# YJxyzxyz/road-vision-system

Measured on AMD Instinct MI355X. Metric: end-to-end frames/sec @1080p (preproc+YOLOv8n+SORT), 1/2/4/8 MI355X, higher is better.
Workload: dtype bf16

## Files before the change

### include/rvhip.h

```cpp
#ifndef RVHIP_H
#define RVHIP_H

#include <stddef.h>
#include <stdint.h>

#ifdef __cplusplus
extern "C" {
#endif

#define RV_OK 0
#define RV_EINVAL (-1000)
#define RV_ECAP (-1001)
#define RV_EOF 1

int rv_abi_version(void);
const char* rv_last_error(void);
int rv_trace_marker(int tag, void* stream);
int rv_install_crash_handler(void);


size_t rv_clahe_ws_bytes(int B, int tiles);

int rv_clahe_ycrcb_u8(const uint8_t* in, uint8_t* out, int B, int H, int W,
                      int pitch, int tiles, double clip, void* ws,
// ... 99 lines not shown
int rv_yolo_pack2(int variant, int dtype, const float* flat, size_t n, void* host_out,
                  size_t out_bytes);
int rv_yolo_create2(int variant, int dtype, const void* dev_packed, int max_B, int in_h, int in_w,
                    void** handle);

int rv_yolo_num_convs_nc(int variant, int nc);
int rv_yolo_conv_info_nc(int variant, int nc, int idx, int* info, char* name, int name_cap);
size_t rv_yolo_flat_floats_nc(int variant, int nc);
size_t rv_yolo_packed_bytes3(int variant, int dtype, int nc);
int rv_yolo_pack3(int variant, int dtype, int nc, const float* flat, size_t n, void* host_out,
                  size_t out_bytes);
int rv_yolo_create3(int variant, int dtype, int nc, const void* dev_packed, int max_B, int in_h,
                    int in_w, void** handle);
int rv_yolo_num_classes(void* handle);
int rv_yolo_head_form(void* handle);
int rv_yolo_set_act_scales(void* handle, const float* scales, int n);
int rv_yolo_buffer_esize(void* handle, int buf);
int rv_yolo_buffer_name(void* handle, int buf, char* name, int cap);
float rv_fp8_scale(double amax);
size_t rv_yolo_ws_bytes(void* handle, int B);
int rv_yolo_num_anchors(void* handle);
int rv_yolo_cand_segments(void* handle);
int rv_yolo_forward(void* handle, const uint8_t* lb, int B, void* ws, size_t ws_bytes,
                    float* raw_out, float conf, void* cand, int cand_cap, int* cand_n,
                    void* stream);
int rv_yolo_forward_part(void* handle, const uint8_t* lb, int B, void* ws, size_t ws_bytes,
                         float* raw_out, float conf, void* cand, int cand_cap, int* cand_n,
                         void* stream, int part);

int rv_yolo_num_buffers(void* handle);
int rv_yolo_buffer_info(void* handle, int B, int buf, int* info, size_t* off_bytes);
int rv_yolo_trace(void* handle, int* recs, int max_recs);
int rv_yolo_attn_trace(void* handle, int* recs, int max_recs);

int rv_yolo_profile(void* handle, int max_forwards);
int rv_yolo_profile_reps(void* handle, int max_forwards, int reps);
int rv_yolo_profile_read(void* handle, double* ms, double* flops, int* conv, int n);
int rv_yolo_profile_bytes(void* handle, double* bytes, int n);
int rv_yolo_profile_times(void* handle, void* ref, double* t0, double* t1, int n);

int rv_yolo_autotune(void* handle, const uint8_t* lb, int B, void* ws, size_t ws_bytes,
                     int reps, int verify, int* n_bad, void* stream);
int rv_yolo_tuned_config(void* handle, int idx, int* cfg6);
int rv_yolo_set_tuned(void* handle, int n, int idx, const int* cfg6);
int rv_yolo_conv_candidates(void* handle, int idx, int* cfg6, int cap);

size_t rv_nms_smem_bytes(void);
int rv_nms_postprocess(const void* cand, const int* seg_n, int B, int cap, int nseg,
                       float iou, int max_det, int max_nms, float max_wh, const float* scale5,
                       const uint32_t* keep_mask4, float* out, int* out_n, int* cand_total,
                       void* ws, size_t ws_bytes, void* stream);
size_t rv_nms_ws_bytes(int B);
int rv_cand_segments(int A);
int rv_candidates_from_raw(const float* raw, int B, int nc, int A, float conf, void* cand,
                           int cap, int* seg_n, void* stream);

size_t rv_sort_state_bytes(int S, int tmax);
size_t rv_sort_ws_bytes(int S, int tmax, int dmax);
int rv_sort_init(void* state, int S, int tmax, void* stream);
int rv_sort_update(void* state_in, void* state_out, int S, int tmax, const float* dets,
                   const int* dcount, int dmax, const double* ts, const double* params6,
                   const double* H9, const float* origin2, void* ws, size_t ws_bytes,
                   int* out_id, double* out_dist, double* out_speed, void* stream);
int rv_sort_stats(const void* state, int S, int* T_out, int* next_id_out, int* overflow_out,
                  void* stream);
int rv_sort_export(const void* state, int S, int tmax, double* x_out, int* meta, int* T_out,
// ... 177 lines not shown
```

### road-vision-system_amd/csrc/c2f.hip

```cpp
#include "conv.h"
#include "conv_common.h"

namespace rv {

typedef __attribute__((ext_vector_type(8))) __bf16 bf16x8c;
typedef __attribute__((ext_vector_type(4))) float f32x4c;
typedef __attribute__((ext_vector_type(2))) float f32x2c;
typedef __attribute__((ext_vector_type(2))) __bf16 bf16x2c;

__device__ __forceinline__ uint32_t c2f_pack(float lo, float hi) {
  return __builtin_bit_cast(uint32_t, __builtin_convertvector(f32x2c{lo, hi}, bf16x2c));
}
__device__ __forceinline__ float c2f_bf2f(uint32_t h) { return __uint_as_float(h << 16); }

template <int C>
struct C2fGeo {
  static constexpr int PB = 2 * C;
  static constexpr int NQ = PB / 16;
  static constexpr int MR = C / 16;
  __device__ static __forceinline__ int addr(int p, int q) { return p * PB + (q << 4); }
};

template <int TR, int TC>
struct C2fTile {
  __host__ __device__ static constexpr int rh(int e) { return TR + 2 * e; }
  __host__ __device__ static constexpr int rw(int e) { return TC + 2 * e; }
  __host__ __device__ static constexpr int rp(int e) { return rh(e) * rw(e); }
};

template <int C, int N, int TR, int TC>
struct C2fLds {
  using G = C2fGeo<C>;
  using T = C2fTile<TR, TC>;
  static constexpr int h = 2 * N;
  static constexpr int Y = 0;
  static constexpr int Tb = Y + T::rp(h) * G::PB;
  static constexpr int Z0 = Tb + T::rp(h - 1) * G::PB;
  static constexpr int Z1 = Z0 + T::rp(h - 2) * G::PB;
  static constexpr int Y0 = Z1 + (N == 2 ? T::rp(0) * G::PB : 0);
  static constexpr int ZR = Y0 + T::rp(0) * G::PB;
  static constexpr int ZBYTES = G::NQ < 4 ? (2 * T::rw(h) + 3) * G::PB : 0;
  static constexpr int BYTES = ZR + ZBYTES;
};

template <int C, int TR, int TC, bool RES, int EO, int ER>
__device__ __forceinline__ void c2f_conv3(const uint8_t* __restrict__ in, uint8_t* __restrict__ outb,
                                          const bf16_t* __restrict__ w,
                                          const float* __restrict__ bias,
                                          const uint8_t* __restrict__ res, int oy0, int ox0, int H,
                                          int W, const uint8_t* __restrict__ zeros, bool pairs) {
  using G = C2fGeo<C>;
  using T = C2fTile<TR, TC>;
  constexpr int MR = G::MR;
  const int tid = threadIdx.x, wave = tid >> 6, lane = tid & 63;
  const int col = lane & 15, quad = lane >> 4;
  constexpr int e_out = EO, e_res = ER;
  constexpr int rwo = T::rw(e_out), rpo = T::rp(e_out), rwi = rwo + 2, rwr = T::rw(e_res);
  bf16x8c A[9][MR];
#pragma unroll
  for (int t = 0; t < 9; ++t)
#pragma unroll
    for (int m = 0; m < MR; ++m)
      A[t][m] = __builtin_bit_cast(bf16x8c,
                                   *(const uint4*)(w + ((size_t)(m * 16 + col) * 9 + t) * 32 + quad * 8));
  f32x4c bv[MR];
#pragma unroll
  for (int m = 0; m < MR; ++m) bv[m] = *(const f32x4c*)(bias + m * 16 + quad * 4);
  const int nfrag = (rpo + 15) / 16;
  if (C == 16 && pairs) {
    bf16x8c Ap[5];
#pragma unroll
    for (int p = 0; p < 5; ++p) {
      const int t = 2 * p + (quad >> 1);
      uint4 v = make_uint4(0, 0, 0, 0);
      if (t < 9) v = *(const uint4*)(w + ((size_t)col * 9 + t) * 32 + (quad & 1) * 8);
      Ap[p] = __builtin_bit_cast(bf16x8c, v);
    }
    const bool hiq = quad >= 2;
    for (int f0 = wave * 2; f0 < nfrag; f0 += 16) {
      f32x4c acc[2];
      int o[2];
      const uint8_t* b1[2];
      const uint8_t* b2[2];
      const uint8_t* b4[2];
#pragma unroll
      for (int n = 0; n < 2; ++n) {
        o[n] = (f0 + n) * 16 + col;
        const int oo = o[n] < rpo ? o[n] : 0;
        const int r = oo / rwo, c = oo - r * rwo;
        const uint8_t* bp = in + G::addr(r * rwi + c, quad & 1);
        b1[n] = bp + (hiq ? G::PB : 0);
        b2[n] = bp + (hiq ? (rwi - 2) * G::PB : 0) + (2 * G::PB);
        b4[n] = hiq ? zeros : bp + (2 * rwi + 2) * G::PB;
        acc[n] = f32x4c{0.f, 0.f, 0.f, 0.f};
      }
      bf16x8c Bp[5][2];
#pragma unroll
      for (int n = 0; n < 2; ++n) {
        Bp[0][n] = __builtin_bit_cast(bf16x8c, *(const uint4*)(b1[n]));
        Bp[1][n] = __builtin_bit_cast(bf16x8c, *(const uint4*)(b2[n]));
        Bp[2][n] = __builtin_bit_cast(bf16x8c, *(const uint4*)(b1[n] + (rwi + 1) * G::PB));
        Bp[3][n] = __builtin_bit_cast(bf16x8c, *(const uint4*)(b1[n] + (2 * rwi) * G::PB));
        Bp[4][n] = __builtin_bit_cast(bf16x8c, *(const uint4*)(b4[n]));
      }
      __builtin_amdgcn_sched_barrier(0);
#pragma unroll
      for (int p = 0; p < 5; ++p)
#pragma unroll
        for (int n = 0; n < 2; ++n)
          acc[n] = __builtin_amdgcn_mfma_f32_16x16x32_bf16(Ap[p], Bp[p][n], acc[n], 0, 0, 0);
#pragma unroll
      for (int n = 0; n < 2; ++n) {
        if (o[n] >= rpo) continue;
        const int r = o[n] / rwo, c = o[n] - (o[n] / rwo) * rwo;
        const int gy = oy0 - e_out + r, gx = ox0 - e_out + c;
        const bool inside = (unsigned)gy < (unsigned)H && (unsigned)gx < (unsigned)W;
        float v[4];
#pragma unroll
        for (int i = 0; i < 4; ++i) v[i] = acc[n][i] + bv[0][i];
        silu4(v);
        const int lq = (quad * 4) >> 3, half = (quad & 1) * 8;
        if (RES) {
          const int d = e_res - e_out;
          const int pr = (r + d) * rwr + c + d;
          const uint2 rr = *(const uint2*)(res + G::addr(pr, lq) + half);
          v[0] += c2f_bf2f(rr.x & 0xFFFF);
          v[1] += c2f_bf2f(rr.x >> 16);
          v[2] += c2f_bf2f(rr.y & 0xFFFF);
          v[3] += c2f_bf2f(rr.y >> 16);
        }
        const uint2 pk = inside ? make_uint2(c2f_pack(v[0], v[1]), c2f_pack(v[2], v[3]))
                                : make_uint2(0, 0);
        *(uint2*)(outb + G::addr(o[n], lq) + half) = pk;
      }
    }
    return;
  }
  for (int f0 = wave * 2; f0 < nfrag; f0 += 16) {
    f32x4c acc[2][MR];
    int o[2];
    const uint8_t* bp[2];
#pragma unroll
    for (int n = 0; n < 2; ++n) {
// ... 26 lines not shown
      __builtin_amdgcn_sched_barrier(0);
    }
#pragma unroll
    for (int n = 0; n < 2; ++n) {
      if (o[n] >= rpo) continue;
      const int r = o[n] / rwo, c = o[n] - (o[n] / rwo) * rwo;
      const int gy = oy0 - e_out + r, gx = ox0 - e_out + c;
      const bool inside = (unsigned)gy < (unsigned)H && (unsigned)gx < (unsigned)W;
#pragma unroll
      for (int m = 0; m < MR; ++m) {
        float v[4];
#pragma unroll
        for (int i = 0; i < 4; ++i) v[i] = acc[n][m][i] + bv[m][i];
        silu4(v);
        const int lq = (m * 16 + quad * 4) >> 3, half = (quad & 1) * 8;
        if (RES) {
          const int d = e_res - e_out;
          const int pr = (r + d) * rwr + c + d;
          const uint2 rr = *(const uint2*)(res + G::addr(pr, lq) + half);
          v[0] += c2f_bf2f(rr.x & 0xFFFF);
          v[1] += c2f_bf2f(rr.x >> 16);
          v[2] += c2f_bf2f(rr.y & 0xFFFF);
          v[3] += c2f_bf2f(rr.y >> 16);
        }
        const uint2 pk = inside ? make_uint2(c2f_pack(v[0], v[1]), c2f_pack(v[2], v[3]))
                                : make_uint2(0, 0);
        *(uint2*)(outb + G::addr(o[n], lq) + half) = pk;
      }
    }
  }
}

template <int C, int N, bool SC, int TR, int TC>
__global__ __launch_bounds__(512) void c2f_chain_kernel(C2fArgs a) {
  extern __shared__ __attribute__((aligned(16))) uint8_t smem[];
  using G = C2fGeo<C>;
  using T = C2fTile<TR, TC>;
  using L = C2fLds<C, N, TR, TC>;
  constexpr int h = 2 * N;
  const int tid = threadIdx.x, wave = tid >> 6, lane = tid & 63;
  const int col = lane & 15, quad = lane >> 4;
  const int tiles_x = (a.W + TC - 1) / TC, tiles_y = (a.H + TR - 1) / TR;
  int bid = blockIdx.x;
  const int tx = bid % tiles_x;
  bid /= tiles_x;
  const int ty = bid % tiles_y;
  const int b = bid / tiles_y;
  const int oy0 = ty * TR, ox0 = tx * TC;
  const bf16_t* img = a.cat + (size_t)b * a.H * a.W * a.cat_cs + a.cat_co;

  {
    constexpr int NY = T::rp(h) * G::NQ, N0 = T::rp(0) * G::NQ;
    constexpr int U1 = (NY + 511) / 512, U0 = (N0 + 511) / 512;
    auto fetch = [&](int i, int n, int e, int rwe, int ch) {
      uint4 v = make_uint4(0, 0, 0, 0);
      if (i < n) {
        const int p = i / G::NQ, q = i - p * G::NQ;
        const int r = p / rwe, c = p - r * rwe;
        const int gy = oy0 - e + r, gx = ox0 - e + c;
        if ((unsigned)gy < (unsigned)a.H && (unsigned)gx < (unsigned)a.W)
          v = *(const uint4*)(img + ((size_t)gy * a.W + gx) * a.cat_cs + ch + q * 8);
      }
      return v;
    };
    uint4 v1[U1], v0[U0];
#pragma unroll
    for (int u = 0; u < U1; ++u) v1[u] = fetch(tid + 512 * u, NY, h, T::rw(h), C);
#pragma unroll
    for (int u = 0; u < U0; ++u) v0[u] = fetch(tid + 512 * u, N0, 0, T::rw(0), 0);
#pragma unroll
    for (int u = 0; u < U1; ++u)
      if (tid + 512 * u < NY) *(uint4*)(smem + L::Y + 16 * (tid + 512 * u)) = v1[u];
#pragma unroll
    for (int u = 0; u < U0; ++u)
      if (tid + 512 * u < N0) *(uint4*)(smem + L::Y0 + 16 * (tid + 512 * u)) = v0[u];
    for (int i = tid; i < L::ZBYTES / 16; i += 512) *(uint4*)(smem + L::ZR + 16 * i) = make_uint4(0, 0, 0, 0);
  }
  __syncthreads();

  const uint8_t* zeros = smem + L::ZR;
  c2f_conv3<C, TR, TC, false, h - 1, 0>(smem + L::Y, smem + L::Tb, a.wa[0], a.ba[0], nullptr, oy0,
                                        ox0, a.H, a.W, zeros, a.tap_pairs != 0);
  __syncthreads();
  c2f_conv3<C, TR, TC, SC, h - 2, h>(smem + L::Tb, smem + L::Z0, a.wb[0], a.bb[0], smem + L::Y, oy0,
                                     ox0, a.H, a.W, zeros, a.tap_pairs != 0);
  __syncthreads();
  if constexpr (N == 2) {
    c2f_conv3<C, TR, TC, false, h - 3, 0>(smem + L::Z0, smem + L::Tb, a.wa[1], a.ba[1], nullptr, oy0,
                                          ox0, a.H, a.W, zeros, a.tap_pairs != 0);
    __syncthreads();
    c2f_conv3<C, TR, TC, SC, h - 4, h - 2>(smem + L::Tb, smem + L::Z1, a.wb[1], a.bb[1],
                                           smem + L::Z0, oy0, ox0, a.H, a.W, zeros, a.tap_pairs != 0);
    __syncthreads();
  }

  constexpr int KC = (2 + N) * C;
  constexpr int NCH = (KC + 31) / 32;
  constexpr int MR2 = 2 * C / 16;
  static_assert(MR2 % 2 == 0, "cv2 stores fragment pairs");
  constexpr int KP = NCH * 32;
  bf16x8c A2[NCH][MR2];
#pragma unroll
  for (int j = 0; j < NCH; ++j)
#pragma unroll
    for (int m = 0; m < MR2; ++m)
      A2[j][m] = __builtin_bit_cast(bf16x8c,
                                    *(const uint4*)(a.w2 + (size_t)(m * 16 + col) * KP + j * 32 + quad * 8));
  f32x4c bv2[MR2];
#pragma unroll
  for (int m = 0; m < MR2; ++m) bv2[m] = *(const f32x4c*)(a.b2 + m * 16 + quad * 4);
  auto seg_buf = [&](int s) -> int {
    return s == 0 ? L::Y0 : (s == 1 ? L::Y : (s == 2 ? L::Z0 : L::Z1));
  };
  auto seg_halo = [&](int s) -> int { return s == 0 ? 0 : (s == 1 ? h : h - 2 * (s - 1)); };
  constexpr int RP0 = T::rp(0);
  constexpr int NFR = RP0 / 16;
  for (int f0 = wave * 2; f0 < NFR; f0 += 16) {
    f32x4c acc[2][MR2];
#pragma unroll
    for (int n = 0; n < 2; ++n)
#pragma unroll
      for (int m = 0; m < MR2; ++m) acc[n][m] = f32x4c{0.f, 0.f, 0.f, 0.f};
    bf16x8c B2[NCH][2];
#pragma unroll
    for (int j = 0; j < NCH; ++j) {
      const int k0 = j * 32 + quad * 8;
      const int s = k0 / C, qq = (k0 - s * C) >> 3;
#pragma unroll
      for (int n = 0; n < 2; ++n) {
        const int o = (f0 + n) * 16 + col;
        const int r = o / TC, c = o - (o / TC) * TC;
        uint4 bq = make_uint4(0, 0, 0, 0);
        if (s < 2 + N) {
          const int e = seg_halo(s);
          const int p = (r + e) * T::rw(e) + c + e;
          bq = *(const uint4*)(smem + seg_buf(s) + G::addr(p, qq));
        }
        B2[j][n] = __builtin_bit_cast(bf16x8c, bq);
      }
    }
    __builtin_amdgcn_sched_barrier(0);
#pragma unroll
    for (int j = 0; j < NCH; ++j)
#pragma unroll
      for (int n = 0; n < 2; ++n)
#pragma unroll
        for (int m = 0; m < MR2; ++m)
          acc[n][m] = __builtin_amdgcn_mfma_f32_16x16x32_bf16(A2[j][m], B2[j][n], acc[n][m], 0, 0, 0);
#pragma unroll
    for (int n = 0; n < 2; ++n) {
      const int o = (f0 + n) * 16 + col;
      const int r = o / TC, c = o - (o / TC) * TC;
      const int gy = oy0 + r, gx = ox0 + c;
      if (gy >= a.H || gx >= a.W) continue;
      uint16_t* dst = a.out + ((size_t)(b * a.H + gy) * a.W + gx) * a.out_cs + a.out_co;
#pragma unroll
      for (int m = 0; m < MR2; m += 2) {
        uint32_t pk[2][2];
#pragma unroll
        for (int h = 0; h < 2; ++h) {
          float v[4];
#pragma unroll
          for (int i = 0; i < 4; ++i) v[i] = acc[n][m + h][i] + bv2[m + h][i];
          silu4(v);
          pk[h][0] = c2f_pack(v[0], v[1]);
          pk[h][1] = c2f_pack(v[2], v[3]);
        }
        const auto x0 = __builtin_amdgcn_permlane16_swap(pk[0][0], pk[1][0], false, false);
        const auto x1 = __builtin_amdgcn_permlane16_swap(pk[0][1], pk[1][1], false, false);
        *(uint4*)(dst + (m + (quad & 1)) * 16 + (quad >> 1) * 8) = make_uint4(x0[0], x1[0], x0[1], x1[1]);
      }
    }
  }
}

template <int C, int N, bool SC, int TR, int TC>
static int launch_c2f_t(const C2fArgs& a, hipStream_t s) {
  using L = C2fLds<C, N, TR, TC>;
  static_assert(L::BYTES <= 160 * 1024, "C2f tile exceeds LDS");
  static_assert((TR * TC) % 32 == 0, "tile must hold whole fragment pairs");
  auto fn = c2f_chain_kernel<C, N, SC, TR, TC>;
  static bool attr = false;
  if (!attr) {
    hipError_t e = hipFuncSetAttribute((const void*)fn, hipFuncAttributeMaxDynamicSharedMemorySize,
                                       L::BYTES);
    if (e != hipSuccess) {
      (void)hipGetLastError();
      set_error("hipFuncSetAttribute(c2f): %s", hipGetErrorString(e));
      return -(int)e;
    }
    attr = true;
  }
  const int blocks = a.B * ceil_div(a.H, TR) * ceil_div(a.W, TC);
  fn<<<blocks, 512, L::BYTES, s>>>(a);
  return launch_status("c2f_chain");
}

bool c2f_fusable(int C, int N, int cat_cs, int cat_co, int out_cs, int out_co) {
  return (C == 16 || C == 32) && (N == 1 || N == 2) && !(C == 16 && N == 2) && cat_cs % 8 == 0 &&
         cat_co % 8 == 0 && out_cs % 4 == 0 && out_co % 4 == 0;
}

int launch_c2f_chain(const C2fArgs& a, int C, int N, bool shortcut, hipStream_t s) {
  if (!c2f_fusable(C, N, a.cat_cs, a.cat_co, a.out_cs, a.out_co)) {
    set_error("c2f_chain: C=%d N=%d unsupported", C, N);
    return RV_EINVAL;
  }
  if (C == 16) return shortcut ? launch_c2f_t<16, 1, true, 16, 32>(a, s)
                               : launch_c2f_t<16, 1, false, 16, 32>(a, s);
  if (N == 1) return shortcut ? launch_c2f_t<32, 1, true, 16, 16>(a, s)
                              : launch_c2f_t<32, 1, false, 16, 16>(a, s);
  return shortcut ? launch_c2f_t<32, 2, true, 16, 16>(a, s) : launch_c2f_t<32, 2, false, 16, 16>(a, s);
}

}
```

### road-vision-system_amd/csrc/conv.h

```cpp
#pragma once
#include "common.h"

namespace rv {

typedef uint16_t bf16_t;

struct ConvArgs {
  const bf16_t* in;
  int in_cs, in_co;
  int Hin, Win, Cin;
  const bf16_t* w;
  const float* bias;
  int Cout, k, stride, pad;
  int Ho, Wo, B;
  void* out0;
  int out0_cs, out0_co, out0_up;
  void* out1;
  int out1_cs, out1_co, out1_up;
  int out_f32;
  const bf16_t* res;
  int res_cs, res_co;
  int act;
  int g2_cout0, g2_in_co, g2_Cin;
  const bf16_t* g2_w;
// ... 27 lines not shown
};
int launch_conv0(const uint8_t* img, int B, int H, int W, const Conv0Q& q, int C0, bf16_t* out,
                 int out_cs, hipStream_t s);
int launch_conv0_fp8(const uint8_t* img, int B, int H, int W, const Conv0Q& q, int C0,
                     uint8_t* out, int out_cs, float s_out, hipStream_t s);

int launch_conv0_k6(const uint8_t* img, int B, int H, int W, const Conv0Q& q, int C0, bf16_t* out,
                    int out_cs, hipStream_t s);

int launch_stem(const uint8_t* img, int B, int H, int W, const Conv0Q& q0, int C0,
                const bf16_t* w1, const float* b1, int C1, bf16_t* out, int out_cs,
                hipStream_t s, const bf16_t* w2 = nullptr, const float* b2 = nullptr,
                bf16_t* out2 = nullptr, int out2_cs = 0, bool k6 = false);

int launch_sppf_pool(bf16_t* buf, int B, int H, int W, int c, hipStream_t s);
int launch_sppf_pool_fp8(uint8_t* buf, int B, int H, int W, int c, hipStream_t s);

struct C2fArgs {
  const bf16_t* cat;
  int cat_cs, cat_co;
  int H, W, B;
  const bf16_t* wa[2];
  const float* ba[2];
  const bf16_t* wb[2];
  const float* bb[2];
  const bf16_t* w2;
  const float* b2;
  bf16_t* out;
  int out_cs, out_co;
  int tap_pairs;
};
bool c2f_fusable(int C, int N, int cat_cs, int cat_co, int out_cs, int out_co);
int launch_c2f_chain(const C2fArgs& a, int C, int N, bool shortcut, hipStream_t s);

int launch_dwconv3x3(const bf16_t* in, int in_cs, int in_co, int in_gw, int in_gs, const bf16_t* w,
                     const float* bias, int B, int H, int W, int C, int act, const bf16_t* res,
                     int res_cs, int res_co, bf16_t* out, int out_cs, int out_co, hipStream_t s);

int launch_psa_attention(const bf16_t* qkv, int B, int N, int heads, int qkv_cs, int qkv_co,
                         bf16_t* out, int out_cs, int out_co, hipStream_t s);

struct HeadLevel {
  const float* logits;
  int H, W, cs;
  float stride;
  const bf16_t* feat;
  int feat_cs, cin_b, cin_c;
  const bf16_t* w_box;
  const bf16_t* w_cls;
  const float* b_box;
  const float* b_cls;
  float* logits_out;
};

struct Cand {
  float x1, y1, x2, y2, score;
  int cls, anchor, pad;
};

int decode_segments(const HeadLevel* lv, int nlv);
int launch_detect_decode(const HeadLevel* lv, int nlv, int B, int nc, int reg_max, float conf,
                         float* raw, Cand* cand, int cand_cap, int* seg_n, hipStream_t s,
                         int* form = nullptr, bool cls_only = false);

struct HeadBoxLevel {
  const bf16_t* t;
// ... 9 lines not shown
```

### road-vision-system_amd/csrc/yolo.hip

```cpp
#include <cmath>
#include <cstring>
#include "yolo_model.h"

namespace rv {

static void plan_heads(Model& M) {
  const Variant& v = M.def.v;
  for (int i = 0; i < 3; ++i) {
    const std::string l = std::to_string(i);
    M.DA[i] = M.newbuf("DA" + l, 3 + i, v.c2d + v.c3p);
    M.DB[i] = M.newbuf("DB" + l, 3 + i, v.c2d + v.c3p, false, true);
    M.HD[i] = M.newbuf("HD" + l, 3 + i, v.hcs, true);
  }
  M.nA = M.map_h[3] * M.map_w[3] + M.map_h[4] * M.map_w[4] + M.map_h[5] * M.map_w[5];
}

static void plan_v5u(Model& M) {
  const Variant& v = M.def.v;
  M.CAT14 = M.CAT11 = -1;
  M.X0 = M.newbuf("X0", 1, v.c1);
  M.X1 = M.newbuf("X1", 2, v.c2);
  M.C2 = M.newbuf("C2", 2, v.c2);
  M.X2 = M.newbuf("X2", 2, v.c2);
  M.X3 = M.newbuf("X3", 3, v.c3);
// ... 1036 lines not shown
  }
  if (segs & 2) {
    if (v11 ? seg_backbone_v11(E) : v5 ? seg_backbone_v5u(E) : seg_backbone(E)) return E.status;
    M->after_neck = here();
  }
  return (segs & 4) ? seg_heads(E, raw_out, conf, cand, cand_cap, cand_n) : RV_OK;
}

extern "C" int rv_yolo_num_buffers(void* h) { return h ? (int)((Model*)h)->bufs.size() : 0; }

extern "C" int rv_yolo_buffer_info(void* h, int B, int buf, int* info, size_t* off_bytes) {
  RV_CHECK_ARG(h && info && off_bytes && B > 0, "bad args");
  Model* M = (Model*)h;
  RV_CHECK_ARG(buf >= 0 && buf < (int)M->bufs.size(), "bad buffer %d", buf);
  *off_bytes = M->offsets(B)[buf];
  const Buf& b = M->bufs[buf];
  info[0] = b.h;
  info[1] = b.w;
  info[2] = b.c;
  info[3] = b.f32 ? 1 : 0;
  return RV_OK;
}

extern "C" int rv_yolo_trace(void* h, int* recs, int max_recs) {
  if (!h) return RV_EINVAL;
  Model* M = (Model*)h;
  const int n = (int)M->trace.size();
  static_assert(sizeof(TraceRec) == 24 * sizeof(int), "rv_yolo_trace: 24 ints per record");
  if (recs)
    for (int i = 0; i < n && i < max_recs; ++i) memcpy(recs + 24 * i, &M->trace[i], 24 * sizeof(int));
  return n;
}

extern "C" int rv_yolo_attn_trace(void* h, int* recs, int max_recs) {
  if (!h) return RV_EINVAL;
  Model* M = (Model*)h;
  const int n = (int)M->attn_trace.size();
  static_assert(sizeof(AttnRec) == 9 * sizeof(int), "rv_yolo_attn_trace: 9 ints per record");
  if (recs)
    for (int i = 0; i < n && i < max_recs; ++i)
      memcpy(recs + 9 * i, &M->attn_trace[i], 9 * sizeof(int));
  return n;
}
```

### road-vision-system_amd/rvs_amd/_lib.py

```python
from __future__ import annotations

import ctypes
import os
from ctypes import c_char_p, c_double, c_float, c_int, c_size_t, c_void_p, POINTER

_HERE = os.path.dirname(os.path.abspath(__file__))
LIB_PATH = os.path.join(_HERE, "librvhip.so")
_variant = os.environ.get("RV_LIB_VARIANT", "default")
if _variant != "default":
    LIB_PATH = os.path.join(_HERE, "librvhip_%s.so" % _variant)

_lib = None


class RVError(RuntimeError):
    """A non-zero status returned through the C ABI."""


_SIGS = {
    "rv_abi_version": (c_int, []),
    "rv_last_error": (ctypes.c_char_p, []),
    "rv_clahe_ws_bytes": (c_size_t, [c_int, c_int]),
    "rv_clahe_ycrcb_u8": (c_int, [c_void_p, c_void_p, c_int, c_int, c_int, c_int, c_int,
                                  c_double, c_void_p, c_size_t, c_void_p]),
# ... 68 lines not shown
    "rv_sink_close": (c_int, [c_void_p]),
    "rv_overlay_ws_bytes": (c_size_t, [c_int, c_int]),
    "rv_overlay_layout": (c_int, [c_void_p, c_void_p, c_void_p, c_void_p, c_void_p, c_int, c_int,
                                  c_int, c_int, c_void_p, c_int, c_int, c_int, c_void_p, c_size_t,
                                  c_void_p]),
    "rv_overlay_raster": (c_int, [c_void_p, c_void_p, c_int, c_int, c_int, c_int, c_int, c_void_p,
                                  c_int, c_void_p, c_void_p, c_void_p]),
    "rv_fog_full_ws_bytes": (c_size_t, [c_int, c_int, c_int]),
    "rv_fog_full_u8": (c_int, [c_void_p, c_void_p, c_int, c_int, c_int, c_int, c_void_p, c_int,
                               c_void_p, c_int, c_void_p, c_void_p, c_void_p, c_void_p,
                               c_void_p, c_void_p, c_int, c_void_p, c_void_p, c_size_t,
                               c_void_p]),
    "rv_letterbox_geometry": (c_int, [c_int, c_int, c_int, c_int, POINTER(c_int)]),
    "rv_letterbox_u8": (c_int, [c_void_p, c_void_p, c_int, c_int, c_int, c_int,
                                POINTER(c_int), c_void_p]),
    "rv_yolo_num_convs": (c_int, [c_int]),
    "rv_yolo_conv_info": (c_int, [c_int, c_int, POINTER(c_int), ctypes.c_char_p, c_int]),
    "rv_yolo_flat_floats": (c_size_t, [c_int]),
    "rv_yolo_packed_bytes": (c_size_t, [c_int]),
    "rv_yolo_pack": (c_int, [c_int, c_void_p, c_size_t, c_void_p, c_size_t]),
    "rv_yolo_create": (c_int, [c_int, c_void_p, c_int, c_int, c_int, POINTER(c_void_p)]),
    "rv_yolo_destroy": (c_int, [c_void_p]),
    "rv_yolo_set_option": (c_int, [c_void_p, c_int, c_int]),
    "rv_conv_bf16": (c_int, [c_void_p, c_int, c_int, c_int, c_int, c_int, c_void_p, c_void_p, c_int,
                             c_int, c_int, c_void_p, c_int, c_void_p, c_int, c_int, c_void_p,
                             c_void_p]),
    "rv_yolo_conv_groups": (c_int, [c_int, c_int, c_int]),
    "rv_dwconv3x3_bf16": (c_int, [c_void_p, c_int, c_int, c_int, c_int, c_int, c_int, c_int, c_int,
                                  c_void_p, c_void_p, c_void_p, c_int, c_int, c_void_p, c_int,
                                  c_int, c_int, c_void_p]),
    "rv_psa_attention_bf16": (c_int, [c_void_p, c_int, c_int, c_int, c_int, c_int, c_void_p, c_int,
                                      c_int, c_void_p]),
    "rv_yolo_attn_trace": (c_int, [c_void_p, c_void_p, c_int]),
    "rv_yolo_packed_bytes2": (c_size_t, [c_int, c_int]),
    "rv_yolo_pack2": (c_int, [c_int, c_int, c_void_p, c_size_t, c_void_p, c_size_t]),
    "rv_yolo_create2": (c_int, [c_int, c_int, c_void_p, c_int, c_int, c_int, POINTER(c_void_p)]),
    "rv_yolo_num_convs_nc": (c_int, [c_int, c_int]),
    "rv_yolo_conv_info_nc": (c_int, [c_int, c_int, c_int, POINTER(c_int), ctypes.c_char_p, c_int]),
    "rv_yolo_flat_floats_nc": (c_size_t, [c_int, c_int]),
    "rv_yolo_packed_bytes3": (c_size_t, [c_int, c_int, c_int]),
    "rv_yolo_pack3": (c_int, [c_int, c_int, c_int, c_void_p, c_size_t, c_void_p, c_size_t]),
    "rv_yolo_create3": (c_int, [c_int, c_int, c_int, c_void_p, c_int, c_int, c_int,
                                POINTER(c_void_p)]),
    "rv_yolo_num_classes": (c_int, [c_void_p]),
    "rv_yolo_head_form": (c_int, [c_void_p]),
    "rv_yolo_set_act_scales": (c_int, [c_void_p, c_void_p, c_int]),
    "rv_yolo_buffer_esize": (c_int, [c_void_p, c_int]),
    "rv_yolo_buffer_name": (c_int, [c_void_p, c_int, ctypes.c_char_p, c_int]),
    "rv_fp8_scale": (c_float, [c_double]),
    "rv_yolo_ws_bytes": (c_size_t, [c_void_p, c_int]),
    "rv_yolo_num_anchors": (c_int, [c_void_p]),
    "rv_yolo_forward": (c_int, [c_void_p, c_void_p, c_int, c_void_p, c_size_t, c_void_p, c_float,
                                c_void_p, c_int, c_void_p, c_void_p]),
    "rv_yolo_forward_part": (c_int, [c_void_p, c_void_p, c_int, c_void_p, c_size_t, c_void_p,
                                     c_float, c_void_p, c_int, c_void_p, c_void_p, c_int]),
    "rv_yolo_num_buffers": (c_int, [c_void_p]),
    "rv_yolo_buffer_info": (c_int, [c_void_p, c_int, c_int, POINTER(c_int), POINTER(c_size_t)]),
    "rv_yolo_trace": (c_int, [c_void_p, c_void_p, c_int]),
    "rv_yolo_profile": (c_int, [c_void_p, c_int]),
    "rv_yolo_profile_reps": (c_int, [c_void_p, c_int, c_int]),
    "rv_yolo_profile_read": (c_int, [c_void_p, c_void_p, c_void_p, c_void_p, c_int]),
    "rv_yolo_profile_bytes": (c_int, [c_void_p, c_void_p, c_int]),
    "rv_yolo_profile_times": (c_int, [c_void_p, c_void_p, c_void_p, c_void_p, c_int]),
    "rv_yolo_autotune": (c_int, [c_void_p, c_void_p, c_int, c_void_p, c_size_t, c_int, c_int,
                                 POINTER(c_int), c_void_p]),
    "rv_yolo_tuned_config": (c_int, [c_void_p, c_int, POINTER(c_int)]),
# ... 51 lines not shown
    lib = ctypes.CDLL(LIB_PATH)
    for name, (res, args) in _SIGS.items():
        if not hasattr(lib, name) and _variant != "default":
            continue
        fn = getattr(lib, name)
        fn.restype = res
        fn.argtypes = args
    _lib = lib
    return lib


def register(name, restype, argtypes):
    _SIGS[name] = (restype, argtypes)
    if _lib is not None:
        fn = getattr(_lib, name)
        fn.restype = restype
        fn.argtypes = argtypes


def check(status: int, what: str = "") -> None:
    if status != 0:
        msg = load().rv_last_error().decode(errors="replace")
        raise RVError(f"{what or 'rvhip'} failed with status {status}: {msg}")


_RECORDABLE = {"rv_clahe_median_letterbox_u8", "rv_clahe_median_u8", "rv_letterbox_u8",
               "rv_yolo_forward_part", "rv_nms_postprocess", "rv_sort_update",
               "rv_results_handback", "rv_untracked_metrics", "rv_preprocess_chain_u8",
               "rv_sort_update_cams", "rv_untracked_metrics_cams"}

_NOCHECK = {"rv_preprocess_chain_route", "rv_sched_num_nodes", "rv_sched_event_query", "rv_abi_version", "rv_cand_segments", "rv_yolo_cand_segments", "rv_clahe_median_fits", "rv_clahe_median_letterbox_fits", "rv_yolo_num_convs", "rv_yolo_num_anchors",
            "rv_yolo_num_buffers", "rv_yolo_trace", "rv_yolo_profile_read", "rv_yolo_tuned_config",
            "rv_yolo_profile_bytes", "rv_yolo_profile_times", "rv_yolo_buffer_esize", "rv_yolo_conv_candidates",
            "rv_yolo_num_classes", "rv_yolo_head_form", "rv_yolo_attn_trace"}


_recorder = None


class recording:

    def __init__(self, sched):
        self.sched = sched

    def __enter__(self):
        global _recorder
        if _recorder is not None:
            raise RuntimeError("a schedule is already being recorded")
        _recorder = self.sched
        return self.sched

    def __exit__(self, *exc):
        global _recorder
        _recorder = None
        return False


def call(name: str, *args) -> int:
    if _recorder is not None and name in _RECORDABLE:
        _recorder.add(name, args)
        return 0
    fn = getattr(load(), name)
    st = fn(*args)
    if fn.restype is c_int and name not in _NOCHECK:
        check(st, name)
    return st

# ... 23 lines not shown
```

Baseline: 46050.

## Make C2f chain kernel persistent with prefetched tiles and LDS-staged weights

For C=32, the fused C2f chain kernel now runs as a persistent grid sized to occupancy times CU count and loops over tiles. The next tile's global input is fetched into registers while the current tile's cv2 stage runs. Some 3x3 conv weights are staged in LDS once per block, the next conv's weights are loaded ahead of the current conv, and cv2 weights are hoisted out of the tile loop. A waves-per-EU hint is added and a plan query API exposes tiles, capacity and grid. The cost is higher LDS and register use, which may lower occupancy.

```diff
diff --git a/include/rvhip.h b/include/rvhip.h
--- a/include/rvhip.h
+++ b/include/rvhip.h
@@ -155,6 +155,7 @@
 int rv_yolo_buffer_info(void* handle, int B, int buf, int* info, size_t* off_bytes);
 int rv_yolo_trace(void* handle, int* recs, int max_recs);
 int rv_yolo_attn_trace(void* handle, int* recs, int max_recs);
+int rv_yolo_c2f_chains(void* handle, int* recs, int max_recs);
 
 int rv_yolo_profile(void* handle, int max_forwards);
 int rv_yolo_profile_reps(void* handle, int max_forwards, int reps);
diff --git a/road-vision-system_amd/csrc/c2f.hip b/road-vision-system_amd/csrc/c2f.hip
--- a/road-vision-system_amd/csrc/c2f.hip
+++ b/road-vision-system_amd/csrc/c2f.hip
@@ -26,6 +26,15 @@
   __host__ __device__ static constexpr int rh(int e) { return TR + 2 * e; }
   __host__ __device__ static constexpr int rw(int e) { return TC + 2 * e; }
   __host__ __device__ static constexpr int rp(int e) { return rh(e) * rw(e); }
+};
+
+template <int C, int N>
+struct C2fPolicy {
+  static constexpr int kLdsConvs = C == 32 ? (N == 1 ? 2 : 1) : 0;
+  static constexpr bool kAhead = C == 32 && N == 2;
+  static constexpr bool kHoistCv2 = C == 32 && N == 1;
+  static constexpr int kMinWaves = C == 16 ? 4 : 2;
+  static constexpr bool kPersistent = C == 32;
 };
 
 template <int C, int N, int TR, int TC>
@@ -40,42 +49,60 @@
   static constexpr int Y0 = Z1 + (N == 2 ? T::rp(0) * G::PB : 0);
   static constexpr int ZR = Y0 + T::rp(0) * G::PB;
   static constexpr int ZBYTES = G::NQ < 4 ? (2 * T::rw(h) + 3) * G::PB : 0;
-  static constexpr int BYTES = ZR + ZBYTES;
-};
-
-template <int C, int TR, int TC, bool RES, int EO, int ER>
-__device__ __forceinline__ void c2f_conv3(const uint8_t* __restrict__ in, uint8_t* __restrict__ outb,
-                                          const bf16_t* __restrict__ w,
-                                          const float* __restrict__ bias,
-                                          const uint8_t* __restrict__ res, int oy0, int ox0, int H,
-                                          int W, const uint8_t* __restrict__ zeros, bool pairs) {
-  using G = C2fGeo<C>;
-  using T = C2fTile<TR, TC>;
-  constexpr int MR = G::MR;
-  const int tid = threadIdx.x, wave = tid >> 6, lane = tid & 63;
+  static constexpr int WL = ZR + ZBYTES;
+  static constexpr int WB = C * 9 * 32 * 2;
+  static constexpr int WBYTES = WB + C * 4;
+  static constexpr int BYTES = WL + C2fPolicy<C, N>::kLdsConvs * WBYTES;
+};
+
+template <int C>
+struct C2fW {
+  bf16x8c A[9][C / 16];
+  f32x4c bv[C / 16];
+};
+
+template <int C>
+__device__ __forceinline__ void c2f_load_w(C2fW<C>& wf, const bf16_t* __restrict__ w,
+                                           const float* __restrict__ bias, bool pairs, int lane) {
+  constexpr int MR = C / 16;
   const int col = lane & 15, quad = lane >> 4;
-  constexpr int e_out = EO, e_res = ER;
-  constexpr int rwo = T::rw(e_out), rpo = T::rp(e_out), rwi = rwo + 2, rwr = T::rw(e_res);
-  bf16x8c A[9][MR];
-#pragma unroll
-  for (int t = 0; t < 9; ++t)
-#pragma unroll
-    for (int m = 0; m < MR; ++m)
-      A[t][m] = __builtin_bit_cast(bf16x8c,
-                                   *(const uint4*)(w + ((size_t)(m * 16 + col) * 9 + t) * 32 + quad * 8));
-  f32x4c bv[MR];
-#pragma unroll
-  for (int m = 0; m < MR; ++m) bv[m] = *(const f32x4c*)(bias + m * 16 + quad * 4);
-  const int nfrag = (rpo + 15) / 16;
   if (C == 16 && pairs) {
-    bf16x8c Ap[5];
 #pragma unroll
     for (int p = 0; p < 5; ++p) {
       const int t = 2 * p + (quad >> 1);
       uint4 v = make_uint4(0, 0, 0, 0);
       if (t < 9) v = *(const uint4*)(w + ((size_t)col * 9 + t) * 32 + (quad & 1) * 8);
-      Ap[p] = __builtin_bit_cast(bf16x8c, v);
-    }
+      wf.A[p][0] = __builtin_bit_cast(bf16x8c, v);
+    }
+  } else {
+#pragma unroll
+    for (int t = 0; t < 9; ++t)
+#pragma unroll
+      for (int m = 0; m < MR; ++m)
+        wf.A[t][m] = __builtin_bit_cast(
+            bf16x8c, *(const uint4*)(w + ((size_t)(m * 16 + col) * 9 + t) * 32 + quad * 8));
+  }
+#pragma unroll
+  for (int m = 0; m < MR; ++m) wf.bv[m] = *(const f32x4c*)(bias + m * 16 + quad * 4);
+}
+
+template <int C, int TR, int TC, bool RES, int EO, int ER>
+__device__ __forceinline__ void c2f_conv3(const uint8_t* __restrict__ in, uint8_t* __restrict__ outb,
+                                          const C2fW<C>& wf,
+                                          const uint8_t* __restrict__ res, int oy0, int ox0, int H,
+                                          int W, const uint8_t* __restrict__ zeros, bool pairs,
+                                          int tid) {
+  using G = C2fGeo<C>;
+  using T = C2fTile<TR, TC>;
+  constexpr int MR = G::MR;
+  const int wave = threadIdx.x >> 6, lane = tid & 63;
+  const int col = lane & 15, quad = lane >> 4;
+  constexpr int e_out = EO, e_res = ER;
+  constexpr int rwo = T::rw(e_out), rpo = T::rp(e_out), rwi = rwo + 2, rwr = T::rw(e_res);
+  const auto& A = wf.A;
+  const auto& bv = wf.bv;
+  const int nfrag = (rpo + 15) / 16;
+  if (C == 16 && pairs) {
     const bool hiq = quad >= 2;
     for (int f0 = wave * 2; f0 < nfrag; f0 += 16) {
       f32x4c acc[2];
@@ -108,7 +135,7 @@
       for (int p = 0; p < 5; ++p)
 #pragma unroll
         for (int n = 0; n < 2; ++n)
-          acc[n] = __builtin_amdgcn_mfma_f32_16x16x32_bf16(Ap[p], Bp[p][n], acc[n], 0, 0, 0);
+          acc[n] = __builtin_amdgcn_mfma_f32_16x16x32_bf16(A[p][0], Bp[p][n], acc[n], 0, 0, 0);
 #pragma unroll
       for (int n = 0; n < 2; ++n) {
         if (o[n] >= rpo) continue;
@@ -201,67 +228,46 @@
 }
 
 template <int C, int N, bool SC, int TR, int TC>
-__global__ __launch_bounds__(512) void c2f_chain_kernel(C2fArgs a) {
+__global__ __launch_bounds__(512)
+__attribute__((amdgpu_waves_per_eu(C2fPolicy<C, N>::kMinWaves))) void c2f_chain_kernel(C2fArgs a) {
   extern __shared__ __attribute__((aligned(16))) uint8_t smem[];
   using G = C2fGeo<C>;
   using T = C2fTile<TR, TC>;
   using L = C2fLds<C, N, TR, TC>;
+  using P = C2fPolicy<C, N>;
   constexpr int h = 2 * N;
   const int tid = threadIdx.x, wave = tid >> 6, lane = tid & 63;
   const int col = lane & 15, quad = lane >> 4;
   const int tiles_x = (a.W + TC - 1) / TC, tiles_y = (a.H + TR - 1) / TR;
-  int bid = blockIdx.x;
-  const int tx = bid % tiles_x;
-  bid /= tiles_x;
-  const int ty = bid % tiles_y;
-  const int b = bid / tiles_y;
-  const int oy0 = ty * TR, ox0 = tx * TC;
-  const bf16_t* img = a.cat + (size_t)b * a.H * a.W * a.cat_cs + a.cat_co;
-
-  {
-    constexpr int NY = T::rp(h) * G::NQ, N0 = T::rp(0) * G::NQ;
-    constexpr int U1 = (NY + 511) / 512, U0 = (N0 + 511) / 512;
+  const int ntiles = tiles_x * tiles_y * a.B;
+  int tile = blockIdx.x;
+  if (tile >= ntiles) return;
+  const bool pairs = a.tap_pairs != 0;
+
+  constexpr int NY = T::rp(h) * G::NQ, N0 = T::rp(0) * G::NQ;
+  constexpr int U1 = (NY + 511) / 512, U0 = (N0 + 511) / 512;
+  uint4 v1[U1], v0[U0];
+  auto fetch_tile = [&](int t, int tid, bool ok) {
+    const int tx = t % tiles_x, ty = (t / tiles_x) % tiles_y, b = t / (tiles_x * tiles_y);
+    const int fy0 = ty * TR, fx0 = tx * TC;
+    const bf16_t* img = a.cat + (size_t)b * a.H * a.W * a.cat_cs + a.cat_co;
     auto fetch = [&](int i, int n, int e, int rwe, int ch) {
       uint4 v = make_uint4(0, 0, 0, 0);
-      if (i < n) {
+      if (ok && i < n) {
         const int p = i / G::NQ, q = i - p * G::NQ;
         const int r = p / rwe, c = p - r * rwe;
-        const int gy = oy0 - e + r, gx = ox0 - e + c;
+        const int gy = fy0 - e + r, gx = fx0 - e + c;
         if ((unsigned)gy < (unsigned)a.H && (unsigned)gx < (unsigned)a.W)
           v = *(const uint4*)(img + ((size_t)gy * a.W + gx) * a.cat_cs + ch + q * 8);
       }
       return v;
     };
-    uint4 v1[U1], v0[U0];
 #pragma unroll
     for (int u = 0; u < U1; ++u) v1[u] = fetch(tid + 512 * u, NY, h, T::rw(h), C);
 #pragma unroll
     for (int u = 0; u < U0; ++u) v0[u] = fetch(tid + 512 * u, N0, 0, T::rw(0), 0);
-#pragma unroll
-    for (int u = 0; u < U1; ++u)
-      if (tid + 512 * u < NY) *(uint4*)(smem + L::Y + 16 * (tid + 512 * u)) = v1[u];
-#pragma unroll
-    for (int u = 0; u < U0; ++u)
-      if (tid + 512 * u < N0) *(uint4*)(smem + L::Y0 + 16 * (tid + 512 * u)) = v0[u];
-    for (int i = tid; i < L::ZBYTES / 16; i += 512) *(uint4*)(smem + L::ZR + 16 * i) = make_uint4(0, 0, 0, 0);
-  }
-  __syncthreads();
-
-  const uint8_t* zeros = smem + L::ZR;
-  c2f_conv3<C, TR, TC, false, h - 1, 0>(smem + L::Y, smem + L::Tb, a.wa[0], a.ba[0], nullptr, oy0,
-                                        ox0, a.H, a.W, zeros, a.tap_pairs != 0);
-  __syncthreads();
-  c2f_conv3<C, TR, TC, SC, h - 2, h>(smem + L::Tb, smem + L::Z0, a.wb[0], a.bb[0], smem + L::Y, oy0,
-                                     ox0, a.H, a.W, zeros, a.tap_pairs != 0);
-  __syncthreads();
-  if constexpr (N == 2) {
-    c2f_conv3<C, TR, TC, false, h - 3, 0>(smem + L::Z0, smem + L::Tb, a.wa[1], a.ba[1], nullptr, oy0,
-                                          ox0, a.H, a.W, zeros, a.tap_pairs != 0);
-    __syncthreads();
-    c2f_conv3<C, TR, TC, SC, h - 4, h - 2>(smem + L::Tb, smem + L::Z1, a.wb[1], a.bb[1],
-                                           smem + L::Z0, oy0, ox0, a.H, a.W, zeros, a.tap_pairs != 0);
-    __syncthreads();
-  }
+  };
+  fetch_tile(tile, tid, true);
 
   constexpr int KC = (2 + N) * C;
   constexpr int NCH = (KC + 31) / 32;
@@ -269,117 +275,240 @@
   static_assert(MR2 % 2 == 0, "cv2 stores fragment pairs");
   constexpr int KP = NCH * 32;
   bf16x8c A2[NCH][MR2];
-#pragma unroll
-  for (int j = 0; j < NCH; ++j)
-#pragma unroll
-    for (int m = 0; m < MR2; ++m)
-      A2[j][m] = __builtin_bit_cast(bf16x8c,
-                                    *(const uint4*)(a.w2 + (size_t)(m * 16 + col) * KP + j * 32 + quad * 8));
   f32x4c bv2[MR2];
-#pragma unroll
-  for (int m = 0; m < MR2; ++m) bv2[m] = *(const f32x4c*)(a.b2 + m * 16 + quad * 4);
-  auto seg_buf = [&](int s) -> int {
-    return s == 0 ? L::Y0 : (s == 1 ? L::Y : (s == 2 ? L::Z0 : L::Z1));
+  auto load_cv2 = [&](int col, int quad) {
+#pragma unroll
+    for (int j = 0; j < NCH; ++j)
+#pragma unroll
+      for (int m = 0; m < MR2; ++m)
+        A2[j][m] = __builtin_bit_cast(
+            bf16x8c, *(const uint4*)(a.w2 + (size_t)(m * 16 + col) * KP + j * 32 + quad * 8));
+#pragma unroll
+    for (int m = 0; m < MR2; ++m) bv2[m] = *(const f32x4c*)(a.b2 + m * 16 + quad * 4);
   };
-  auto seg_halo = [&](int s) -> int { return s == 0 ? 0 : (s == 1 ? h : h - 2 * (s - 1)); };
-  constexpr int RP0 = T::rp(0);
-  constexpr int NFR = RP0 / 16;
-  for (int f0 = wave * 2; f0 < NFR; f0 += 16) {
-    f32x4c acc[2][MR2];
-#pragma unroll
-    for (int n = 0; n < 2; ++n)
-#pragma unroll
-      for (int m = 0; m < MR2; ++m) acc[n][m] = f32x4c{0.f, 0.f, 0.f, 0.f};
-    bf16x8c B2[NCH][2];
-#pragma unroll
-    for (int j = 0; j < NCH; ++j) {
-      const int k0 = j * 32 + quad * 8;
-      const int s = k0 / C, qq = (k0 - s * C) >> 3;
+  if (P::kHoistCv2) load_cv2(col, quad);
+  if constexpr (P::kLdsConvs > 0) {
+    const bf16_t* wsrc[2] = {a.wa[0], a.wb[0]};
+    const float* bsrc[2] = {a.ba[0], a.bb[0]};
+#pragma unroll
+    for (int k = 0; k < P::kLdsConvs; ++k) {
+      uint8_t* dst = smem + L::WL + k * L::WBYTES;
+      for (int i = tid; i < L::WB / 16; i += 512) *(uint4*)(dst + 16 * i) = ((const uint4*)wsrc[k])[i];
+      if (tid < C / 4) *(uint4*)(dst + L::WB + 16 * tid) = ((const uint4*)bsrc[k])[tid];
+    }
+  }
+  auto load_lds_w = [&](C2fW<C>& wf, int k, int ti) {
+    const uint8_t* src = smem + L::WL + k * L::WBYTES;
+    c2f_load_w<C>(wf, (const bf16_t*)src, (const float*)(src + L::WB), false, ti & 63);
+  };
+  for (int i = tid; i < L::ZBYTES / 16; i += 512) *(uint4*)(smem + L::ZR + 16 * i) = make_uint4(0, 0, 0, 0);
+  const uint8_t* zeros = smem + L::ZR;
+  C2fW<C> w0, w1;
+
+  for (;;) {
+    const int tx = tile % tiles_x, ty = (tile / tiles_x) % tiles_y, b = tile / (tiles_x * tiles_y);
+    const int oy0 = ty * TR, ox0 = tx * TC;
+    int ti = tid;
+    asm volatile("" : "+v"(ti));
+    const int col = ti & 15, quad = (ti & 63) >> 4;
+#pragma unroll
+    for (int u = 0; u < U1; ++u)
+      if (tid + 512 * u < NY) *(uint4*)(smem + L::Y + 16 * (tid + 512 * u)) = v1[u];
+#pragma unroll
+    for (int u = 0; u < U0; ++u)
+      if (tid + 512 * u < N0) *(uint4*)(smem + L::Y0 + 16 * (tid + 512 * u)) = v0[u];
+    __syncthreads();
+
+    if constexpr (P::kAhead) {
+      static_assert(N == 2 && P::kLdsConvs == 1, "the ahead form: four phases, the first from LDS");
+      load_lds_w(w0, 0, ti);
+      c2f_load_w<C>(w1, a.wb[0], a.bb[0], pairs, ti & 63);
+      c2f_conv3<C, TR, TC, false, h - 1, 0>(smem + L::Y, smem + L::Tb, w0, nullptr, oy0, ox0, a.H,
+                                            a.W, zeros, pairs, ti);
+      __syncthreads();
+      c2f_load_w<C>(w0, a.wa[1], a.ba[1], pairs, ti & 63);
+      c2f_conv3<C, TR, TC, SC, h - 2, h>(smem + L::Tb, smem + L::Z0, w1, smem + L::Y, oy0, ox0, a.H,
+                                         a.W, zeros, pairs, ti);
+      __syncthreads();
+      c2f_load_w<C>(w1, a.wb[1], a.bb[1], pairs, ti & 63);
+      c2f_conv3<C, TR, TC, false, h - 3, 0>(smem + L::Z0, smem + L::Tb, w0, nullptr, oy0, ox0, a.H,
+                                            a.W, zeros, pairs, ti);
+      __syncthreads();
+      load_cv2(col, quad);
+      c2f_conv3<C, TR, TC, SC, h - 4, h - 2>(smem + L::Tb, smem + L::Z1, w1, smem + L::Z0, oy0, ox0,
+                                             a.H, a.W, zeros, pairs, ti);
+      __syncthreads();
+    } else {
+      auto load_w = [&](int k, const bf16_t* w, const float* bias) {
+        if (k < P::kLdsConvs) load_lds_w(w0, k, ti);
+        else c2f_load_w<C>(w0, w, bias, pairs, ti & 63);
+      };
+      load_w(0, a.wa[0], a.ba[0]);
+      c2f_conv3<C, TR, TC, false, h - 1, 0>(smem + L::Y, smem + L::Tb, w0, nullptr, oy0, ox0, a.H,
+                                            a.W, zeros, pairs, ti);
+      __syncthreads();
+      load_w(1, a.wb[0], a.bb[0]);
+      c2f_conv3<C, TR, TC, SC, h - 2, h>(smem + L::Tb, smem + L::Z0, w0, smem + L::Y, oy0, ox0, a.H,
+                                         a.W, zeros, pairs, ti);
+      __syncthreads();
+      if constexpr (N == 2) {
+        load_w(2, a.wa[1], a.ba[1]);
+        c2f_conv3<C, TR, TC, false, h - 3, 0>(smem + L::Z0, smem + L::Tb, w0, nullptr, oy0, ox0, a.H,
+                                              a.W, zeros, pairs, ti);
+        __syncthreads();
+        load_w(3, a.wb[1], a.bb[1]);
+        c2f_conv3<C, TR, TC, SC, h - 4, h - 2>(smem + L::Tb, smem + L::Z1, w0, smem + L::Z0, oy0,
+                                               ox0, a.H, a.W, zeros, pairs, ti);
+        __syncthreads();
+      }
+    }
+
+    const int next = tile + gridDim.x;
+    fetch_tile(next, ti, next < ntiles);
+    if (!P::kHoistCv2 && !P::kAhead) load_cv2(col, quad);
+    auto seg_buf = [&](int s) -> int {
+      return s == 0 ? L::Y0 : (s == 1 ? L::Y : (s == 2 ? L::Z0 : L::Z1));
+    };
+    auto seg_halo = [&](int s) -> int { return s == 0 ? 0 : (s == 1 ? h : h - 2 * (s - 1)); };
+    constexpr int RP0 = T::rp(0);
+    constexpr int NFR = RP0 / 16;
+    for (int f0 = wave * 2; f0 < NFR; f0 += 16) {
+      f32x4c acc[2][MR2];
+#pragma unroll
+      for (int n = 0; n < 2; ++n)
+#pragma unroll
+        for (int m = 0; m < MR2; ++m) acc[n][m] = f32x4c{0.f, 0.f, 0.f, 0.f};
+      bf16x8c B2[NCH][2];
+#pragma unroll
+      for (int j = 0; j < NCH; ++j) {
+        const int k0 = j * 32 + quad * 8;
+        const int s = k0 / C, qq = (k0 - s * C) >> 3;
+#pragma unroll
+        for (int n = 0; n < 2; ++n) {
+          const int o = (f0 + n) * 16 + col;
+          const int r = o / TC, c = o - (o / TC) * TC;
+          uint4 bq = make_uint4(0, 0, 0, 0);
+          if (s < 2 + N) {
+            const int e = seg_halo(s);
+            const int p = (r + e) * T::rw(e) + c + e;
+            bq = *(const uint4*)(smem + seg_buf(s) + G::addr(p, qq));
+          }
+          B2[j][n] = __builtin_bit_cast(bf16x8c, bq);
+        }
+      }
+      __builtin_amdgcn_sched_barrier(0);
+#pragma unroll
+      for (int j = 0; j < NCH; ++j)
+#pragma unroll
+        for (int n = 0; n < 2; ++n)
+#pragma unroll
+          for (int m = 0; m < MR2; ++m)
+            acc[n][m] = __builtin_amdgcn_mfma_f32_16x16x32_bf16(A2[j][m], B2[j][n], acc[n][m], 0, 0, 0);
 #pragma unroll
       for (int n = 0; n < 2; ++n) {
         const int o = (f0 + n) * 16 + col;
         const int r = o / TC, c = o - (o / TC) * TC;
-        uint4 bq = make_uint4(0, 0, 0, 0);
-        if (s < 2 + N) {
-          const int e = seg_halo(s);
-          const int p = (r + e) * T::rw(e) + c + e;
-          bq = *(const uint4*)(smem + seg_buf(s) + G::addr(p, qq));
+        const int gy = oy0 + r, gx = ox0 + c;
+        if (gy >= a.H || gx >= a.W) continue;
+        uint16_t* dst = a.out + ((size_t)(b * a.H + gy) * a.W + gx) * a.out_cs + a.out_co;
+#pragma unroll
+        for (int m = 0; m < MR2; m += 2) {
+          uint32_t pk[2][2];
+#pragma unroll
+          for (int h = 0; h < 2; ++h) {
+            float v[4];
+#pragma unroll
+            for (int i = 0; i < 4; ++i) v[i] = acc[n][m + h][i] + bv2[m + h][i];
+            silu4(v);
+            pk[h][0] = c2f_pack(v[0], v[1]);
+            pk[h][1] = c2f_pack(v[2], v[3]);
+          }
+          const auto x0 = __builtin_amdgcn_permlane16_swap(pk[0][0], pk[1][0], false, false);
+          const auto x1 = __builtin_amdgcn_permlane16_swap(pk[0][1], pk[1][1], false, false);
+          *(uint4*)(dst + (m + (quad & 1)) * 16 + (quad >> 1) * 8) = make_uint4(x0[0], x1[0], x0[1], x1[1]);
         }
-        B2[j][n] = __builtin_bit_cast(bf16x8c, bq);
-      }
-    }
-    __builtin_amdgcn_sched_barrier(0);
-#pragma unroll
-    for (int j = 0; j < NCH; ++j)
-#pragma unroll
-      for (int n = 0; n < 2; ++n)
-#pragma unroll
-        for (int m = 0; m < MR2; ++m)
-          acc[n][m] = __builtin_amdgcn_mfma_f32_16x16x32_bf16(A2[j][m], B2[j][n], acc[n][m], 0, 0, 0);
-#pragma unroll
-    for (int n = 0; n < 2; ++n) {
-      const int o = (f0 + n) * 16 + col;
-      const int r = o / TC, c = o - (o / TC) * TC;
-      const int gy = oy0 + r, gx = ox0 + c;
-      if (gy >= a.H || gx >= a.W) continue;
-      uint16_t* dst = a.out + ((size_t)(b * a.H + gy) * a.W + gx) * a.out_cs + a.out_co;
-#pragma unroll
-      for (int m = 0; m < MR2; m += 2) {
-        uint32_t pk[2][2];
-#pragma unroll
-        for (int h = 0; h < 2; ++h) {
-          float v[4];
-#pragma unroll
-          for (int i = 0; i < 4; ++i) v[i] = acc[n][m + h][i] + bv2[m + h][i];
-          silu4(v);
-          pk[h][0] = c2f_pack(v[0], v[1]);
-          pk[h][1] = c2f_pack(v[2], v[3]);
-        }
-        const auto x0 = __builtin_amdgcn_permlane16_swap(pk[0][0], pk[1][0], false, false);
-        const auto x1 = __builtin_amdgcn_permlane16_swap(pk[0][1], pk[1][1], false, false);
-        *(uint4*)(dst + (m + (quad & 1)) * 16 + (quad >> 1) * 8) = make_uint4(x0[0], x1[0], x0[1], x1[1]);
-      }
-    }
-  }
-}
+      }
+    }
+    if (next >= ntiles) break;
+    tile = next;
+    __syncthreads();
+  }
+}
+
+struct C2fPlan {
+  int tiles, capacity, grid;
+};
 
 template <int C, int N, bool SC, int TR, int TC>
-static int launch_c2f_t(const C2fArgs& a, hipStream_t s) {
+struct C2fInst {
   using L = C2fLds<C, N, TR, TC>;
   static_assert(L::BYTES <= 160 * 1024, "C2f tile exceeds LDS");
   static_assert((TR * TC) % 32 == 0, "tile must hold whole fragment pairs");
-  auto fn = c2f_chain_kernel<C, N, SC, TR, TC>;
-  static bool attr = false;
-  if (!attr) {
-    hipError_t e = hipFuncSetAttribute((const void*)fn, hipFuncAttributeMaxDynamicSharedMemorySize,
-                                       L::BYTES);
-    if (e != hipSuccess) {
+
+  static int plan(const C2fArgs& a, C2fPlan& p) {
+    auto fn = c2f_chain_kernel<C, N, SC, TR, TC>;
+    static int occ = 0;
+    if (!occ) {
+      hipError_t e = hipFuncSetAttribute((const void*)fn, hipFuncAttributeMaxDynamicSharedMemorySize,
+                                         L::BYTES);
+      if (e != hipSuccess) {
+        (void)hipGetLastError();
+        set_error("hipFuncSetAttribute(c2f): %s", hipGetErrorString(e));
+        return -(int)e;
+      }
+      int o = 0;
+      if (hipOccupancyMaxActiveBlocksPerMultiprocessor(&o, fn, 512, L::BYTES) != hipSuccess || o < 1)
+        o = 1;
       (void)hipGetLastError();
-      set_error("hipFuncSetAttribute(c2f): %s", hipGetErrorString(e));
-      return -(int)e;
-    }
-    attr = true;
-  }
-  const int blocks = a.B * ceil_div(a.H, TR) * ceil_div(a.W, TC);
-  fn<<<blocks, 512, L::BYTES, s>>>(a);
-  return launch_status("c2f_chain");
-}
+      occ = o;
+    }
+    p.tiles = a.B * ceil_div(a.H, TR) * ceil_div(a.W, TC);
+    p.capacity = occ * num_cus();
+    p.grid = C2fPolicy<C, N>::kPersistent ? std::min(p.tiles, p.capacity) : p.tiles;
+    return RV_OK;
+  }
+
+  static int launch(const C2fArgs& a, hipStream_t s) {
+    C2fPlan p;
+    if (const int st = plan(a, p)) return st;
+    c2f_chain_kernel<C, N, SC, TR, TC><<<p.grid, 512, L::BYTES, s>>>(a);
+    return launch_status("c2f_chain");
+  }
+};
 
 bool c2f_fusable(int C, int N, int cat_cs, int cat_co, int out_cs, int out_co) {
   return (C == 16 || C == 32) && (N == 1 || N == 2) && !(C == 16 && N == 2) && cat_cs % 8 == 0 &&
          cat_co % 8 == 0 && out_cs % 4 == 0 && out_co % 4 == 0;
 }
 
+template <class F>
+static int c2f_dispatch(int C, int N, bool shortcut, F&& f) {
+  if (C == 16) return shortcut ? f(C2fInst<16, 1, true, 16, 32>{}) : f(C2fInst<16, 1, false, 16, 32>{});
+  if (N == 1) return shortcut ? f(C2fInst<32, 1, true, 16, 16>{}) : f(C2fInst<32, 1, false, 16, 16>{});
+  return shortcut ? f(C2fInst<32, 2, true, 16, 16>{}) : f(C2fInst<32, 2, false, 16, 16>{});
+}
+
+static bool c2f_check(const C2fArgs& a, int C, int N) {
+  if (c2f_fusable(C, N, a.cat_cs, a.cat_co, a.out_cs, a.out_co)) return true;
+  set_error("c2f_chain: C=%d N=%d unsupported", C, N);
+  return false;
+}
+
 int launch_c2f_chain(const C2fArgs& a, int C, int N, bool shortcut, hipStream_t s) {
-  if (!c2f_fusable(C, N, a.cat_cs, a.cat_co, a.out_cs, a.out_co)) {
-    set_error("c2f_chain: C=%d N=%d unsupported", C, N);
-    return RV_EINVAL;
-  }
-  if (C == 16) return shortcut ? launch_c2f_t<16, 1, true, 16, 32>(a, s)
-                               : launch_c2f_t<16, 1, false, 16, 32>(a, s);
-  if (N == 1) return shortcut ? launch_c2f_t<32, 1, true, 16, 16>(a, s)
-                              : launch_c2f_t<32, 1, false, 16, 16>(a, s);
-  return shortcut ? launch_c2f_t<32, 2, true, 16, 16>(a, s) : launch_c2f_t<32, 2, false, 16, 16>(a, s);
-}
-
-}
+  if (!c2f_check(a, C, N)) return RV_EINVAL;
+  return c2f_dispatch(C, N, shortcut, [&](auto inst) { return decltype(inst)::launch(a, s); });
+}
+
+int c2f_chain_plan(const C2fArgs& a, int C, int N, bool shortcut, int* tiles, int* capacity,
+                   int* grid) {
+  if (!c2f_check(a, C, N)) return RV_EINVAL;
+  C2fPlan p{};
+  const int st =
+      c2f_dispatch(C, N, shortcut, [&](auto inst) { return decltype(inst)::plan(a, p); });
+  *tiles = p.tiles;
+  *capacity = p.capacity;
+  *grid = p.grid;
+  return st;
+}
+
+}
diff --git a/road-vision-system_amd/csrc/conv.h b/road-vision-system_amd/csrc/conv.h
--- a/road-vision-system_amd/csrc/conv.h
+++ b/road-vision-system_amd/csrc/conv.h
@@ -83,6 +83,8 @@
 };
 bool c2f_fusable(int C, int N, int cat_cs, int cat_co, int out_cs, int out_co);
 int launch_c2f_chain(const C2fArgs& a, int C, int N, bool shortcut, hipStream_t s);
+int c2f_chain_plan(const C2fArgs& a, int C, int N, bool shortcut, int* tiles, int* capacity,
+                   int* grid);
 
 int launch_dwconv3x3(const bf16_t* in, int in_cs, int in_co, int in_gw, int in_gs, const bf16_t* w,
                      const float* bias, int B, int H, int W, int C, int act, const bf16_t* res,
diff --git a/road-vision-system_amd/csrc/yolo.hip b/road-vision-system_amd/csrc/yolo.hip
--- a/road-vision-system_amd/csrc/yolo.hip
+++ b/road-vision-system_amd/csrc/yolo.hip
@@ -1092,6 +1092,19 @@
   return n;
 }
 
+extern "C" int rv_yolo_c2f_chains(void* h, int* recs, int max_recs) {
+  if (!h) return RV_EINVAL;
+  Model* M = (Model*)h;
+  const int n = (int)M->fused.size();
+  for (int i = 0; recs && i < n && i < max_recs; ++i) {
+    const Model::FusedC2f& f = M->fused[i];
+    int* r = recs + 6 * i;
+    r[0] = f.C, r[1] = f.N, r[2] = f.shortcut;
+    if (const int st = c2f_chain_plan(f.a, f.C, f.N, f.shortcut, r + 3, r + 4, r + 5)) return st;
+  }
+  return n;
+}
+
 extern "C" int rv_yolo_attn_trace(void* h, int* recs, int max_recs) {
   if (!h) return RV_EINVAL;
   Model* M = (Model*)h;
diff --git a/road-vision-system_amd/rvs_amd/_lib.py b/road-vision-system_amd/rvs_amd/_lib.py
--- a/road-vision-system_amd/rvs_amd/_lib.py
+++ b/road-vision-system_amd/rvs_amd/_lib.py
@@ -124,6 +124,7 @@
     "rv_psa_attention_bf16": (c_int, [c_void_p, c_int, c_int, c_int, c_int, c_int, c_void_p, c_int,
                                       c_int, c_void_p]),
     "rv_yolo_attn_trace": (c_int, [c_void_p, c_void_p, c_int]),
+    "rv_yolo_c2f_chains": (c_int, [c_void_p, c_void_p, c_int]),
     "rv_yolo_packed_bytes2": (c_size_t, [c_int, c_int]),
     "rv_yolo_pack2": (c_int, [c_int, c_int, c_void_p, c_size_t, c_void_p, c_size_t]),
     "rv_yolo_create2": (c_int, [c_int, c_int, c_void_p, c_int, c_int, c_int, POINTER(c_void_p)]),
@@ -241,7 +242,7 @@
 _NOCHECK = {"rv_preprocess_chain_route", "rv_sched_num_nodes", "rv_sched_event_query", "rv_abi_version", "rv_cand_segments", "rv_yolo_cand_segments", "rv_clahe_median_fits", "rv_clahe_median_letterbox_fits", "rv_yolo_num_convs", "rv_yolo_num_anchors",
             "rv_yolo_num_buffers", "rv_yolo_trace", "rv_yolo_profile_read", "rv_yolo_tuned_config",
             "rv_yolo_profile_bytes", "rv_yolo_profile_times", "rv_yolo_buffer_esize", "rv_yolo_conv_candidates",
-            "rv_yolo_num_classes", "rv_yolo_head_form", "rv_yolo_attn_trace"}
+            "rv_yolo_num_classes", "rv_yolo_head_form", "rv_yolo_attn_trace", "rv_yolo_c2f_chains"}
 
 
 _recorder = None
```

Result: no change. 45830 (-0.5%).
